# vanTeeffelenLab/ExTrack

Measured on AMD Instinct MI355X. Metric: log-likelihood evals/sec (1e6 tracks, 2-state, len=30), higher is better.
Workload: dtype f64

## Files before the change

### extrack_amd/csrc/xt_fast2.h

```cpp
#pragma once
#include "xt_kernel.h"

#define XT_F2_CHUNK 32
#ifndef XT_F2_RENORM
#define XT_F2_RENORM 3
#endif
#define XT_F2_WAVES 4

static inline bool xt_use_fast2(int S, int NS, int F, bool preds) { return S == 2 && NS == 1 && F >= 4 && F <= 7 && !preds; }

template <int F>
struct XtF2Geom {
    static constexpr int E = 1 << F;
    static constexpr int NG = E / 2;
    static constexpr int TPW = 64 / NG;
    static constexpr int EW = E * TPW;
};

template <int F>
XT_HD int xt_f2_swz(int w)
{
    const int c4[7] = {0x5, 0x12, 0x14, 0x2c, 0x4f, 0x41, 0x15};
    const int c6[7] = {0x15, 0x36, 0x67, 0x1c, 0x2, 0x1a, 0x16};
    const int c7[7] = {0x65, 0x72, 0x6, 0x69, 0x1c, 0x4, 0x5f};
    int s = 0;
    for (int j = 0; j < 7; ++j) {
        const int col = F == 6 ? c6[j] : (F == 7 ? c7[j] : c4[j]);
        s ^= ((w >> j) & 1) ? col : 0;
    }
    return s;
}

#define XT_F2_XCLAMP XT_TCLAMP
#define XT_F2_EXP_ENTRIES 1024
#define XT_F2_EXP_BYTES (XT_F2_EXP_ENTRIES * 8)
#define XT_F2_EXP_SCALE 1477.3197218702985
#define XT_F2_EXP_HI (-6.769015308236703e-04)
#define XT_F2_EXP_LO (-1.2691901263564344e-11)
#define XT_F2_EXP_C2 0.5000000047728719
XT_HD void xt_f2_exp_bits(double t, int& j, int& e)
{
    union {
        double d;
        unsigned long long u;
    } v;
    v.d = t;
    j = (int)(v.u & (XT_F2_EXP_ENTRIES - 1));
    e = (int)(unsigned int)(v.u >> 10);
}
XT_HD void xt_exp_tab_x2(double x0, double x1, double& p0, double& p1, int& j0, int& j1, int& e0, int& e1)
{
    x0 = x0 > XT_F2_XCLAMP ? x0 : XT_F2_XCLAMP;
    x1 = x1 > XT_F2_XCLAMP ? x1 : XT_F2_XCLAMP;
    const double t0 = xt_fma(x0, XT_F2_EXP_SCALE, XT_MAGIC);
    const double t1 = xt_fma(x1, XT_F2_EXP_SCALE, XT_MAGIC);
    const double k0 = t0 - XT_MAGIC;
    const double k1 = t1 - XT_MAGIC;
    double r0 = xt_fma(k0, XT_F2_EXP_HI, x0);
    double r1 = xt_fma(k1, XT_F2_EXP_HI, x1);
    r0 = xt_fma(k0, XT_F2_EXP_LO, r0);
    r1 = xt_fma(k1, XT_F2_EXP_LO, r1);
    double q0 = 1.66666666666666666667e-01, q1 = 1.66666666666666666667e-01;
#define XT_H2(C)              \
    q0 = xt_fma(q0, r0, (C)); \
    q1 = xt_fma(q1, r1, (C));
    XT_H2(XT_F2_EXP_C2)
    XT_H2(1.0)
    XT_H2(1.0)
#undef XT_H2
    p0 = q0;
    p1 = q1;
    xt_f2_exp_bits(t0, j0, e0);
    xt_f2_exp_bits(t1, j1, e1);
}
XT_HD void xt_exp_tab_x1(double x, double& p, int& j, int& e)
{
    x = x > XT_F2_XCLAMP ? x : XT_F2_XCLAMP;
    const double t = xt_fma(x, XT_F2_EXP_SCALE, XT_MAGIC);
    const double k = t - XT_MAGIC;
    double r = xt_fma(k, XT_F2_EXP_HI, x);
    r = xt_fma(k, XT_F2_EXP_LO, r);
#if defined(__HIP_DEVICE_COMPILE__)
    double q;
    asm("v_fma_f64 %0, %1, %2, %3" : "=v"(q) : "s"(1.66666666666666666667e-01), "v"(r), "v"(XT_F2_EXP_C2));
#else
    double q = xt_fma(1.66666666666666666667e-01, r, XT_F2_EXP_C2);
#endif
    q = xt_fma(q, r, 1.0);
    p = xt_fma(q, r, 1.0);
    xt_f2_exp_bits(t, j, e);
}
template <class Ctx>
XT_HD void xt_f2_build_exp_table(Ctx& cx, char* lds, int off, const double* T64)
{
    for (int i = cx.tid(); i < XT_F2_EXP_ENTRIES; i += cx.nthreads()) {
        const double sv = (double)(i & 15) * (XT_LN2 / 1024.0);
        double q = 1.0 / 5040.0;
        q = xt_fma(q, sv, 1.0 / 720.0);
        q = xt_fma(q, sv, 1.0 / 120.0);
        q = xt_fma(q, sv, 1.0 / 24.0);
        q = xt_fma(q, sv, 1.0 / 6.0);
        q = xt_fma(q, sv, 0.5);
        q = xt_fma(q, sv, 1.0);
        q = xt_fma(q, sv, 1.0);
        *(double*)(lds + off + i * 8) = T64[i >> 4] * q;
    }
}

template <int F, int D, int K>
struct XtF2State {
    int s01[F];
};

#define XT_F2_EXPB_OFF 1024
#define XT_F2_TAB_BYTES (1024 + XT_F2_EXP_BYTES)
#define XT_F2_T64_OFF ((XT_BLOB_HDR + XT_NTAB * 4) * 8)
#define XT_F2_NAN_OFF 832
#define XT_F2_ARR (XT_F2_WAVES * 128 * 8)
#define XT_F2_ZM0 XT_F2_TAB_BYTES
XT_HD int xt_f2_ze0(int D, int K) { return XT_F2_ZM0 + (1 + D + K) * XT_F2_ARR; }
XT_HD int xt_f2_pos0(int D, int K) { return xt_f2_ze0(D, K) + XT_F2_ARR; }
XT_HD int xt_f2_acc0(int D, int K, int KS, int tpw) { return xt_f2_pos0(D, K) + XT_F2_WAVES * tpw * XT_F2_CHUNK * (D + KS) * 8; }
XT_HD int xt_f2_block_bytes(int D, int K, int KS, int tpw) { return xt_f2_acc0(D, K, KS, tpw) + XT_F2_WAVES * 8 * 3 * 8; }

XT_HD int xt_opaque(int v)
{
#if defined(__HIP_DEVICE_COMPILE__)
    asm volatile("" : "+v"(v));
#endif
    return v;
}

template <class T>
XT_HD T& xt_at(char* lds, int byte_off)
{
#if defined(__HIP_DEVICE_COMPILE__)
    (void)lds;
    return *(__attribute__((address_space(3))) T*)(unsigned int)byte_off;
#else
    return *(T*)(lds + byte_off);
#endif
}
XT_HD void xt_f2_check_lds_base(char* lds)
{
#if defined(__HIP_DEVICE_COMPILE__)
    if ((unsigned int)(unsigned long long)(__attribute__((address_space(3))) char*)lds != 0u) __builtin_trap();
#else
    (void)lds;
#endif
}

template <int F, int D, int K, int H, bool ZF = false, bool LAZY = false>
XT_HD void xt_f2_step(char* lds, const XtF2State<F, D, K>& st, const double* c, const double* l2, const double* TT, const double* TD2)
{
    constexpr int ZEO = (1 + D + K) * XT_F2_ARR;
    const int pk = xt_opaque(st.s01[H]);
    const int a0 = pk & 0xffff, a1 = (int)((unsigned)pk >> 16);
    const double z0 = xt_at<double>(lds, a0), z1 = xt_at<double>(lds, a1);
    const int e0 = xt_at<int>(lds, a0 + ZEO), e1 = xt_at<int>(lds, a1 + ZEO);
    const int emax = e0 > e1 ? e0 : e1;
    const double w0 = xt_ldexp(z0, e0 - emax), w1 = xt_ldexp(z1, e1 - emax);
    const double W = w0 + w1;
    double M[D], U[K];
    for (int d = 0; d < D; ++d)
        M[d] = xt_fma(w1, xt_at<double>(lds, a1 + (1 + d) * XT_F2_ARR), w0 * xt_at<double>(lds, a0 + (1 + d) * XT_F2_ARR));
    for (int k = 0; k < K; ++k)
        U[k] = xt_fma(w1, xt_at<double>(lds, a1 + (1 + D + k) * XT_F2_ARR), w0 * xt_at<double>(lds, a0 + (1 + D + k) * XT_F2_ARR));
    const bool live = ZF ? true : W > 0.0;
    const double Ws = ZF ? W : (live ? W : 1.0);
    constexpr bool RN = !LAZY || (H % XT_F2_RENORM) == 0;
    const double Wm = RN ? xt_frexp_mant(W) : W;
    const int We = live ? (RN ? emax + xt_frexp_exp(W) : emax) : XT_EMIN;

    double Dq[2][K];
    for (int q = 0; q < 2; ++q)
        for (int k = 0; k < K; ++k) Dq[q][k] = xt_fma(Ws, l2[k] + TD2[q], U[k]);
    double rD[2][K], rW;
    if (K == 1) {
        const double d01 = Dq[0][0] * Dq[1][0];
        const double R = xt_rcp(Ws * d01);
        const double RW = R * Ws;
        rW = R * d01;
        rD[0][0] = RW * Dq[1][0];
        rD[1][0] = RW * Dq[0][0];
    } else {
        double f[2 * K + 1], pre[2 * K + 2], suf[2 * K + 2];
        f[0] = Ws;
        for (int q = 0; q < 2; ++q)
            for (int k = 0; k < K; ++k) f[1 + q * K + k] = Dq[q][k];
        pre[0] = 1.0;
        for (int i = 0; i < 2 * K + 1; ++i) pre[i + 1] = pre[i] * f[i];
        suf[2 * K + 1] = 1.0;
        for (int i = 2 * K; i >= 0; --i) suf[i] = suf[i + 1] * f[i];
        const double R = xt_rcp(pre[2 * K + 1]);
        rW = R * suf[1];
        for (int q = 0; q < 2; ++q)
            for (int k = 0; k < K; ++k) rD[q][k] = R * pre[1 + q * K + k] * suf[2 + q * K + k];
    }
    double dmW[D], dsqW = 0.0;
    for (int d = 0; d < D; ++d) {
        dmW[d] = xt_fma(c[d], Ws, -M[d]);
        if (K == 1) dsqW = xt_fma(dmW[d], dmW[d], dsqW);
    }
    double x[2], gf[2], tt[2][K];
    const double A = -0.5 * rW * dsqW;
    for (int q = 0; q < 2; ++q) {
        if (K == 1) {
            x[q] = A * rD[q][0];
            tt[q][0] = xt_fma(Ws, TD2[q], U[0]) * rD[q][0];
            gf[q] = xt_pow_half<D>(Ws * rD[q][0]);
        } else {
            double xx = 0.0, gg = 1.0;
            for (int d = 0; d < D; ++d) {
                xx = xt_fma(dmW[d] * dmW[d], rD[q][d], xx);
                tt[q][d] = xt_fma(Ws, TD2[q], U[d]) * rD[q][d];
                gg *= Ws * rD[q][d];
            }
            x[q] = xx * (-0.5 * rW);
            gf[q] = sqrt(gg);
        }
    }
    double p[2];
    int j[2], n[2];
    xt_exp_tab_x2(x[0], x[1], p[0], p[1], j[0], j[1], n[0], n[1]);
    for (int q = 0; q < 2; ++q) {
        const int aq = q ? a1 : a0;
        int en = We + n[q];
        const double tj = xt_at<double>(lds, XT_F2_EXPB_OFF + j[q] * 8);
        double zn = (Wm * TT[q]) * (gf[q] * tj) * p[q];
        if (!LAZY) {
            en += xt_frexp_exp(zn);
            zn = xt_frexp_mant(zn);
        }
        xt_at<double>(lds, aq) = zn;
        xt_at<int>(lds, aq + ZEO) = en > XT_EMIN ? en : XT_EMIN;
        for (int d = 0; d < D; ++d) xt_at<double>(lds, aq + (1 + d) * XT_F2_ARR) = xt_fma(dmW[d], tt[q][K == 1 ? 0 : d], M[d]) * rW;
        for (int k = 0; k < K; ++k) xt_at<double>(lds, aq + (1 + D + k) * XT_F2_ARR) = l2[k] * tt[q][k];
    }
}

template <int F, int D, int K, class Ctx>
// ... 232 lines not shown
```

### extrack_amd/csrc/xt_reg2.h

```cpp
#pragma once
#include "xt_fast2.h"
#include "xt_grad.h"


template <int F>
struct XtR2Geom {
    static constexpr int NGB = F - 1;
    static constexpr int NG = 1 << NGB;
    static constexpr int TPW = 64 / NG;
};
XT_HD constexpr int xt_r2_gbit(int F, int i) { return F == 7 ? i : (i < 2 ? i : i + 1); }
XT_HD constexpr int xt_r2_gmask(int F) { return F == 7 ? 63 : (F == 6 ? 0x3b : (F == 5 ? 0x1b : 0x0b)); }
template <int F>
XT_HD int xt_r2_slot(int lane)
{
    if (F == 7) return 0;
    int ts = (lane >> 2) & 1;
    if (F == 5) ts |= ((lane >> 5) & 1) << 1;
    if (F == 4) ts |= ((lane >> 4) & 3) << 1;
    return ts;
}

#define XT_R2_TAN0 XT_F2_TAB_BYTES
#define XT_R2_TB 36
// ... 124 lines not shown
        int en = We + n[q];
        const double tj = xt_at<double>(lds, XT_F2_EXPB_OFF + j[q] * 8);
        double zn = (Wm * TT[q]) * (gf[q] * tj) * p[q];
        if (!LAZY) {
            en += xt_frexp_exp(zn);
            zn = xt_frexp_mant(zn);
        }
        nz[q] = zn;
        ne[q] = en > XT_EMIN ? en : XT_EMIN;
        XT_UNROLL
        for (int d = 0; d < D; ++d) nm[q][d] = xt_fma(dmW[d], tt[q][K == 1 ? 0 : d], M[d]) * rW;
        XT_UNROLL
        for (int k = 0; k < K; ++k) nu[q][k] = l2[k] * tt[q][k];
    }

    double a0 = 0.0, a1 = 0.0, cm[D], cu[K], dn[D], Aq[2][K], rq[2][K];
    if (NP > 0) {
        a0 = w0 * rW;
        a1 = w1 * rW;
        const double aa = a0 * a1;
        XT_UNROLL
        for (int d = 0; d < D; ++d) {
            cm[d] = aa * (s.m[0][d] - s.m[1][d]);
            dn[d] = dmW[d] * rW;
        }
        XT_UNROLL
        for (int k = 0; k < K; ++k) cu[k] = aa * (s.u[0][k] - s.u[1][k]);
        XT_UNROLL
        for (int q = 0; q < 2; ++q)
            XT_UNROLL
            for (int k = 0; k < K; ++k) {
                rq[q][k] = Ws * rD[q][k];
                if (K == 1)
                    Aq[q][0] = -0.5 * rq[q][0] * xt_fma(-(dsqW * rW * rW), rq[q][0], (double)D);
                else
                    Aq[q][k] = -0.5 * rq[q][k] * xt_fma(-(dn[k] * dn[k]), rq[q][k], 1.0);
            }
    }
    cx.template pair_exchange<XB>(nz[0], nz[1]);
    cx.template pair_exchange_i32<XB>(ne[0], ne[1]);
    XT_UNROLL
    for (int d = 0; d < D; ++d) cx.template pair_exchange<XB>(nm[0][d], nm[1][d]);
    XT_UNROLL
    for (int k = 0; k < K; ++k) cx.template pair_exchange<XB>(nu[0][k], nu[1][k]);
    XT_UNROLL
    for (int q = 0; q < 2; ++q) {
        s.z[q] = nz[q];
        s.e[q] = ne[q];
        XT_UNROLL
        for (int d = 0; d < D; ++d) s.m[q][d] = nm[q][d];
        XT_UNROLL
        for (int k = 0; k < K; ++k) s.u[q][k] = nu[q][k];
    }
    if (NP > 0) {
        XT_UNROLL
        for (int pp = 0; pp < NP; ++pp) {
            if (!(VAR & 1)) xt_sched_fence();
            const int tb = XT_R2_TAN0 + pp * XT_R2_TB * 8;
            double dl[K];
            XT_UNROLL
            for (int k = 0; k < K; ++k) dl[k] = xt_at<double>(lds, tb + k * 8);
            const double del = s.rz[pp][0] - s.rz[pp][1];
            const double R = xt_fma(a0, s.rz[pp][0], a1 * s.rz[pp][1]);
            double dmb[D], dub[K];
            XT_UNROLL
            for (int d = 0; d < D; ++d) dmb[d] = xt_fma(cm[d], del, xt_fma(a0, s.dm[pp][0][d], a1 * s.dm[pp][1][d]));
            XT_UNROLL
            for (int k = 0; k < K; ++k) dub[k] = xt_fma(cu[k], del, xt_fma(a0, s.du[pp][0][k], a1 * s.du[pp][1][k]));
            double hd[K];
            if (K == 1) {
                hd[0] = 0.0;
                XT_UNROLL
                for (int d = 0; d < D; ++d) hd[0] = xt_fma(dn[d], dmb[d], hd[0]);
            } else {
                XT_UNROLL
                for (int d = 0; d < D; ++d) hd[d] = dn[d] * dmb[d];
            }
            double trz[2], tdm[2][D], tdu[2][K];
            XT_UNROLL
            for (int q = 0; q < 2; ++q) {
                const double dlT = xt_at<double>(lds, tb + tab + io[q]);
                const double dd2 = xt_at<double>(lds, tb + XT_R2_TAB0 + 4 * 32 + io[q]);
                double rzn = R + dlT, dtt[K];
                XT_UNROLL
                for (int k = 0; k < K; ++k) {
                    const double ds2 = dd2 + dub[k], dden = dl[k] + ds2;
                    dtt[k] = rq[q][k] * xt_fma(-tt[q][k], dden, ds2);
                    rzn = xt_fma(Aq[q][k], dden, rzn);
                    rzn = xt_fma(rq[q][k], hd[k], rzn);
                    tdu[q][k] = xt_fma(l2[k], dtt[k], dl[k] * tt[q][k]);
                }
                trz[q] = ZF ? rzn : (live ? rzn : 0.0);
                XT_UNROLL
                for (int d = 0; d < D; ++d) {
                    const int kk = K == 1 ? 0 : d;
                    tdm[q][d] = xt_fma(dn[d], dtt[kk], xt_fma(-tt[q][kk], dmb[d], dmb[d]));
                }
            }
            cx.template pair_exchange<XB>(trz[0], trz[1]);
            XT_UNROLL
            for (int d = 0; d < D; ++d) cx.template pair_exchange<XB>(tdm[0][d], tdm[1][d]);
            XT_UNROLL
            for (int k = 0; k < K; ++k) cx.template pair_exchange<XB>(tdu[0][k], tdu[1][k]);
            XT_UNROLL
            for (int q = 0; q < 2; ++q) {
                s.rz[pp][q] = trz[q];
                XT_UNROLL
                for (int d = 0; d < D; ++d) s.dm[pp][q][d] = tdm[q][d];
                XT_UNROLL
                for (int k = 0; k < K; ++k) s.du[pp][q][k] = tdu[q][k];
            }
        }
    }
}

#ifndef XT_R2_RC_H
#define XT_R2_RC_H 0
#endif
#define XT_R2_RC_NONE (-2147483647 - 1)
#define XT_R2_IO_BITS 5
template <int F, int H, class Ctx>
XT_HD int xt_r2_pack_io(int lane)
{
    constexpr int NGB = F - 1;
    if constexpr (H >= NGB) {
        return 0;
    } else {
        constexpr int XB = xt_r2_gbit(F, H), PB = xt_r2_gbit(F, (H + NGB - 1) % NGB);
        const int prev = (lane >> PB) & 1;
        const int qa = Ctx::template pair_natural<XB>() ? 0 : (lane >> XB) & 1;
        return ((prev * 2 + qa) * 8) << (XT_R2_IO_BITS * H) | xt_r2_pack_io<F, H + 1, Ctx>(lane);
    }
}
XT_HD void xt_r2_opaque_inplace(int& pk)
{
#if defined(__HIP_DEVICE_COMPILE__)
    asm volatile("" : "+v"(pk));
#else
    (void)pk;
#endif
}
template <class Ctx>
XT_HD int xt_r2_tid8(Ctx& cx)
{
#if defined(__HIP_DEVICE_COMPILE__)
    int o;
    asm volatile("v_lshlrev_b32 %0, 3, %1" : "=v"(o) : "v"(cx.tid()));
    return o;
#else
    return cx.tid() * 8;
#endif
}
template <int F, int D, int H, bool FIRST = false, class Ctx>
XT_HD void xt_r2_step_g(Ctx& cx, char* lds, XtR2Lane<D, 1, 0>& s, double (&lx)[2], int& pk, int tab, const double* c)
{
    constexpr int NGB = F - 1;
    constexpr int XB = xt_r2_gbit(F, H);
    xt_r2_opaque_inplace(pk);
    int io0 = (int)(((unsigned int)pk >> (XT_R2_IO_BITS * H)) & ((1u << XT_R2_IO_BITS) - 1u));
    xt_r2_opaque_inplace(io0);
    const int io[2] = {io0, io0 ^ 8};
    double TD2[2], LT[2];
    XT_UNROLL
    for (int q = 0; q < 2; ++q) {
        TD2[q] = xt_at<double>(lds, XT_R2_TAB0 + 4 * 32 + io[q]);
        LT[q] = xt_at<double>(lds, tab + XT_R2_LNT_REL + io[q]);
    }
    const double l2 = xt_at<double>(lds, 0), l22 = xt_at<double>(lds, XT_R2_GC_OFF + 8);

    double w0 = 1.0, w1 = 0.0, base = lx[0];
    if (!FIRST) {
        const double dl = lx[1] - lx[0];
        double p;
        int j, n;
        xt_exp_tab_x1(-fabs(dl), p, j, n);
        const double E = xt_ldexp(xt_at<double>(lds, XT_F2_EXPB_OFF + j * 8) * p, n);
        const bool up = dl > 0.0;
        w0 = s.z[0] * (up ? E : 1.0);
        w1 = s.z[1] * (up ? 1.0 : E);
        base = up ? lx[1] : lx[0];
    }
    const double Ws = FIRST ? 1.0 : w0 + w1;
    double M[D];
    XT_UNROLL
    for (int d = 0; d < D; ++d) M[d] = FIRST ? s.m[0][d] : xt_fma(w1, s.m[1][d], w0 * s.m[0][d]);
    const double V = FIRST ? s.u[0][0] : xt_fma(w1, s.u[1][0], w0 * s.u[0][0]);
    constexpr bool RN = !FIRST && (H % XT_F2_RENORM) == 0;
    const double Wm = FIRST ? s.z[0] : (RN ? xt_frexp_mant(Ws) : Ws);
    if (RN) base = xt_fma((double)xt_frexp_exp(Ws), XT_LN2, base);
    if (!FIRST && H == XT_R2_RC_H) {
        const int tid8 = xt_r2_tid8(cx);
        const int rc0 = xt_r2_rc0(D, 0, XtR2Geom<F>::TPW);
        const int cell = rc0 + (tid8 & ~(xt_r2_gmask(F) * 8));
        cx.atomic_max_i32(&xt_at<int>(lds, cell), (int)fmin(fmax(base, -1e9), 1e9));
        cx.wave_sync();
        const int sh = xt_at<int>(lds, cell);
        base -= (double)sh;
        xt_at<unsigned int>(lds, rc0 + XT_R2_RC_ARR + tid8) += (unsigned int)sh;
    }
    if (!FIRST && H == (XT_R2_RC_H + 1) % NGB) xt_at<int>(lds, xt_r2_rc0(D, 0, XtR2Geom<F>::TPW) + (xt_r2_tid8(cx) & ~(xt_r2_gmask(F) * 8))) = XT_R2_RC_NONE;

    const double Dq0 = xt_fma(Ws, TD2[0], V), Dq1 = xt_fma(Ws, TD2[1], V);
    const double R = xt_rcp3(Ws * (Dq0 * Dq1));
    const double h[2] = {R * Dq1, R * Dq0};
    const double l2W = FIRST ? l2 : l2 * Ws;
    double ed[D], esq = 0.0;
    XT_UNROLL
    for (int d = 0; d < D; ++d) {
        ed[d] = FIRST ? c[d] - M[d] : xt_fma(c[d], Ws, -M[d]);
        esq = xt_fma(ed[d], ed[d], esq);
    }
    const double Ah = -0.5 * esq;
    const double WmW = FIRST ? Wm : Wm * Ws;
    double ny[2], nl[2], nm[2][D], nv[2];
    XT_UNROLL
    for (int q = 0; q < 2; ++q) {
        const double k = l2W * h[q];
        ny[q] = D == 2 ? WmW * k : Wm * xt_pow_half<D>(FIRST ? k : Ws * k);
        nl[q] = xt_fma(Ah, h[q], LT[q]) + base;
        XT_UNROLL
        for (int d = 0; d < D; ++d) nm[q][d] = xt_fma(-ed[d], k, c[d]);
        nv[q] = xt_fma(-l2W, k, l22);
    }
    cx.template pair_exchange<XB>(ny[0], ny[1]);
    cx.template pair_exchange<XB>(nl[0], nl[1]);
    XT_UNROLL
    for (int d = 0; d < D; ++d) cx.template pair_exchange<XB>(nm[0][d], nm[1][d]);
    cx.template pair_exchange<XB>(nv[0], nv[1]);
    XT_UNROLL
    for (int q = 0; q < 2; ++q) {
        s.z[q] = ny[q];
        lx[q] = nl[q];
        XT_UNROLL
        for (int d = 0; d < D; ++d) s.m[q][d] = nm[q][d];
        s.u[q][0] = nv[q];
    }
}

template <int F, class Ctx>
XT_HD double xt_r2_gsum(Ctx& cx, double v)
{
    constexpr int NGB = F - 1;
    v += cx.template xor_f64<xt_r2_gbit(F, 0)>(v);
    v += cx.template xor_f64<xt_r2_gbit(F, 1)>(v);
    v += cx.template xor_f64<xt_r2_gbit(F, 2)>(v);
    if (NGB > 3) v += cx.template xor_f64<xt_r2_gbit(F, NGB > 3 ? 3 : 0)>(v);
    if (NGB > 4) v += cx.template xor_f64<xt_r2_gbit(F, NGB > 4 ? 4 : 0)>(v);
    if (NGB > 5) v += cx.template xor_f64<xt_r2_gbit(F, NGB > 5 ? 5 : 0)>(v);
    return v;
}
template <int F, class Ctx>
XT_HD int xt_r2_gmax(Ctx& cx, int v)
{
    constexpr int NGB = F - 1;
    auto mx = [](int a, int b) XT_INL { return a > b ? a : b; };
    v = mx(v, cx.template xor_i32<xt_r2_gbit(F, 0)>(v));
    v = mx(v, cx.template xor_i32<xt_r2_gbit(F, 1)>(v));
    v = mx(v, cx.template xor_i32<xt_r2_gbit(F, 2)>(v));
    if (NGB > 3) v = mx(v, cx.template xor_i32<xt_r2_gbit(F, NGB > 3 ? 3 : 0)>(v));
    if (NGB > 4) v = mx(v, cx.template xor_i32<xt_r2_gbit(F, NGB > 4 ? 4 : 0)>(v));
    if (NGB > 5) v = mx(v, cx.template xor_i32<xt_r2_gbit(F, NGB > 5 ? 5 : 0)>(v));
    return v;
}

template <int F, int D, int K, int NP, class Ctx, class GetPos>
XT_HD void xt_r2_chain(Ctx& cx, char* lds, XtR2Lane<D, K, NP>& s, int T, int stay_from, GetPos& getpos)
{
    constexpr int NGB = F - 1;
    const int lane = xt_opaque(cx.lane());
    double z = s.z[0];
    int e = s.e[0];
    XT_UNROLL
    for (int t = 1; t < NGB; ++t) {
        if (t > T) break;
        const int prev = (lane >> xt_r2_gbit(F, t == 1 ? NGB - 1 : t - 2)) & 1;
        const int q = (lane >> xt_r2_gbit(F, t - 1)) & 1;
        const int io = (prev * 2 + q) * 8;
        const double TT = xt_at<double>(lds, XT_R2_TAB0 + (t >= stay_from ? 32 : 0) + io);
        const double d2 = xt_at<double>(lds, XT_R2_TAB0 + 4 * 32 + io);
        double c[D], l2[K];
        getpos(t, c, l2);
        double tt[K], r[K], dm[D], x = 0.0, gf;
        XT_UNROLL
        for (int k = 0; k < K; ++k) {
            const double a = d2 + s.u[0][k];
            r[k] = NP == 0 ? xt_rcp3(l2[k] + a) : xt_rcp(l2[k] + a);
            tt[k] = a * r[k];
        }
        XT_UNROLL
        for (int d = 0; d < D; ++d) dm[d] = c[d] - s.m[0][d];
        if (K == 1) {
            XT_UNROLL
            for (int d = 0; d < D; ++d) x = xt_fma(dm[d], dm[d], x);
            x *= -0.5 * r[0];
            gf = xt_pow_half<D>(r[0]);
        } else {
            double gg = 1.0;
            XT_UNROLL
            for (int d = 0; d < D; ++d) {
                x = xt_fma(-0.5 * dm[d] * dm[d], r[d], x);
                gg *= r[d];
            }
            gf = sqrt(gg);
        }
        double p;
        int j, n;
        xt_exp_tab_x1(x, p, j, n);
        z = (z * TT) * (gf * xt_at<double>(lds, XT_F2_EXPB_OFF + j * 8)) * p;
        e += n;
        XT_UNROLL
        for (int d = 0; d < D; ++d) s.m[0][d] = xt_fma(dm[d], tt[K == 1 ? 0 : d], s.m[0][d]);
        XT_UNROLL
        for (int k = 0; k < K; ++k) s.u[0][k] = l2[k] * tt[k];
    }
    int dummy = 0;
    XT_UNROLL
    for (int i = 0; i < NGB - 1; ++i)
        if (i >= T) dummy |= 1 << xt_r2_gbit(F, i);
    const bool live = (lane & dummy) == 0;
    s.z[0] = live ? xt_frexp_mant(z) : 0.0;
    s.e[0] = live ? e + xt_frexp_exp(z) : XT_EMIN;
}

template <int F, int D, int K, int NP, int VAR = 0, class Ctx>
XT_HD void xt_r2_body(const XtKernelArgs& a, const XtGradArgs& ga, Ctx& cx)
{
    int lb, nb;
    const XtBucketDesc b = xt_bind_bucket(a, cx.block(), cx.nblocks(), lb, nb);
    typedef XtR2Geom<F> Gm;
    constexpr int NGB = Gm::NGB, TPW = Gm::TPW;
    constexpr int GMASK = xt_r2_gmask(F);
    const int lane = cx.lane();
    const int wib = NP == 0 ? cx.uniform(cx.wave_in_block()) : cx.wave_in_block();
    const int nwb = cx.waves_per_block();
    const int L = b.L;
    const int KS = a.locerr_mode ? a.KS : 0;
    double* smem = cx.smem();
    char* lds = (char*)smem;

    const int ntab = xt_tab_doubles(2, 2);
    for (int i = cx.tid(); i < ntab; i += cx.nthreads()) smem[i] = xt_blob_ptr(a)[i];
    if (NP > 0)
        for (int i = cx.tid(); i < NP * XT_R2_TB; i += cx.nthreads()) xt_at<double>(lds, XT_R2_TAN0 + i * 8) = ga.dblob[i];
    const int NU = NP > 0 ? ga.NU : 0, NPT = NP + NU;
    for (int i = cx.tid(); i < NU * XT_R2_TB; i += cx.nthreads()) xt_at<double>(lds, XT_R2_TAN0 + (NP * XT_R2_TB + i) * 8) = ga.udblob[i];
    cx.sync();
    xt_f2_check_lds_base(lds);
    xt_f2_build_exp_table(cx, lds, XT_F2_EXPB_OFF, (const double*)(lds + XT_F2_T64_OFF));
    const bool gform = NP == 0 && K == 1 && a.well_scaled == 2 && a.locerr_mode == 0;
    if constexpr (NP == 0 && K == 1) {
        if (gform && cx.tid() < 10) {
            const int i = cx.tid();
            const double l2 = smem[0];
            if (i < 8)
                xt_at<double>(lds, XT_R2_LNT_OFF + i * 8) = log(smem[XT_BLOB_HDR + i]) - 0.5 * D * log(l2);
            else
                xt_at<double>(lds, XT_R2_GC_OFF + (i - 8) * 8) = i == 8 ? -0.5 / l2 : 2.0 * l2;
        }
    }
    cx.sync();
    const double* hdr = smem;

    const int ts = xt_r2_slot<F>(lane);
    const bool leader = (lane & GMASK) == 0;
    const int tlast = L - 1;
    const int stay_from = a.min_len > 2 ? a.min_len : 2;
    const int vfin = (b.isBL ? 2 : 0) + (tlast >= stay_from ? 1 : 0);
    double l2g[K];
    XT_UNROLL
    for (int k = 0; k < K; ++k) l2g[k] = hdr[k];
    int pk = xt_r2_pack_io<F, 0, Ctx>(lane);
    const bool well_scaled = a.well_scaled != 0;
    const bool chain = NP == 0 && well_scaled;

    double* pos = (double*)(lds + xt_r2_pos0(NPT)) + wib * TPW * XT_F2_CHUNK * (D + KS);
    double* sig = pos + TPW * XT_F2_CHUNK * D;
    const int posb = NP == 0 ? xt_opaque(xt_r2_pos0(0) + (wib * TPW * XT_F2_CHUNK * (D + KS) + ts * XT_F2_CHUNK * D) * 8) : 0;
    double* accp = (double*)(lds + xt_r2_acc0(NPT, D, KS, TPW)) + (wib * 8 + ts) * (NPT + 3);
    auto accb = [&]() XT_INL { return xt_r2_acc0(0, D, KS, TPW) + (wib * 8 + xt_r2_slot<F>(xt_opaque(cx.lane()))) * 24; };
    auto rcacc = [&]() XT_INL { return xt_r2_rc0(D, KS, TPW) + XT_R2_RC_ARR + xt_opaque(cx.tid()) * 8; };
    auto rcsum = [&]() XT_INL { return xt_r2_rc0(D, KS, TPW) + 2 * XT_R2_RC_ARR + (wib * 8 + xt_r2_slot<F>(xt_opaque(cx.lane()))) * 8; };
    if (leader) {
        if (NP == 0) {
            const int ab = accb();
            xt_at<double>(lds, ab) = 1.0;
            xt_at<double>(lds, ab + 8) = 0.0;
            xt_at<double>(lds, ab + 16) = 0.0;
            xt_at<double>(lds, rcsum()) = 0.0;
        } else {
            for (int i = 0; i < NPT + 1; ++i) accp[i] = 0.0;
        }
    }

    const int64_t nbatch = (b.N + TPW - 1) / TPW;
    const int64_t W0 = (int64_t)lb * nwb + wib, NW = (int64_t)nb * nwb;
    for (int64_t batch = W0; batch < nbatch; batch += NW) {
        const int64_t trk = batch * TPW + ts;
        const bool act = trk < b.N;

        auto stage = [&](int p0) XT_INL {
            cx.wave_sync();
            for (int i = lane; i < TPW * XT_F2_CHUNK * D; i += 64) {
                const int t_ = i / (XT_F2_CHUNK * D), r = i - t_ * (XT_F2_CHUNK * D);
                const int64_t tk = batch * TPW + t_;
                const int64_t tkc = tk < b.N ? tk : b.N - 1;
                const int pp = p0 + r / D;
                if (pp < L) {
                    const double v = b.tracks[(tkc * L + p0) * D + r];
                    pos[i] = v;
                    if (v != v) xt_at<int>(lds, XT_F2_NAN_OFF + (wib * 8 + t_) * 4) = 1;
                }
            }
            if (KS)
                for (int i = lane; i < TPW * XT_F2_CHUNK * KS; i += 64) {
                    const int t_ = i / (XT_F2_CHUNK * KS), r = i - t_ * (XT_F2_CHUNK * KS);
                    const int64_t tk = batch * TPW + t_;
                    const int64_t tkc = tk < b.N ? tk : b.N - 1;
                    const int pp = p0 + r / KS;
                    if (pp < L) {
                        const double v = b.sigma[(tkc * L + p0) * KS + r];
                        sig[i] = v;
                        if (v != v) xt_at<int>(lds, XT_F2_NAN_OFF + (wib * 8 + t_) * 4) = 1;
                    }
                }
            cx.wave_sync();
        };
        auto getpos = [&](int t, double* c, double* l2) XT_INL {
            const int r = t & (XT_F2_CHUNK - 1);
            XT_UNROLL
            for (int d = 0; d < D; ++d) c[d] = NP == 0 ? xt_at<double>(lds, posb + (r * D + d) * 8) : pos[(ts * XT_F2_CHUNK + r) * D + d];
            if (KS == 0) {
                XT_UNROLL
                for (int k = 0; k < K; ++k) l2[k] = xt_at<double>(lds, k * 8);
            } else {
                XT_UNROLL
                for (int k = 0; k < K; ++k) {
                    double sg = sig[(ts * XT_F2_CHUNK + r) * KS + (KS == 1 ? 0 : k)];
                    if (a.locerr_mode == 2) {
                        sg = xt_fma(sg, hdr[3], hdr[4]);
                        sg = sg < 1e-6 ? 1e-6 : sg;
                    }
                    l2[k] = sg * sg;
                }
            }
        };

        XtR2Lane<D, K, NP> s;
        double lx[2] = {0.0, 0.0};
#define XT_R2_PHASE(H, ZF_, LAZY_)                                                                     \
    if (NGB > (H) && t <= tend2 && ph == (H)) {                                                        \
        double c[D], l2[K];                                                                            \
        getpos(t, c, l2);                                                                              \
        xt_r2_step<F, D, K, NP, ((H) < NGB ? (H) : 0), ZF_, LAZY_, VAR>(cx, lds, s, XT_R2_TABSEL, c, l2);   \
        ++t;                                                                                           \
        ph = (H) + 1 == NGB ? 0 : (H) + 1;                                                             \
    }
#define XT_R2_PHASE_G(H)                                                                               \
    if (NGB > (H) && t <= tend2 && ph == (H)) {                                                        \
        double c[D], l2[K];                                                                            \
        getpos(t, c, l2);                                                                              \
        xt_r2_step_g<F, D, ((H) < NGB ? (H) : 0)>(cx, lds, s, lx, pk, XT_R2_TABSEL, c);                    \
        ++t;                                                                                           \
        ph = (H) + 1 == NGB ? 0 : (H) + 1;                                                             \
    }
#define XT_R2_PHASES(ZF_, LAZY_) \
    XT_R2_PHASE(0, ZF_, LAZY_)   \
    XT_R2_PHASE(1, ZF_, LAZY_)   \
    XT_R2_PHASE(2, ZF_, LAZY_)   \
    XT_R2_PHASE(3, ZF_, LAZY_)   \
    XT_R2_PHASE(4, ZF_, LAZY_)   \
    XT_R2_PHASE(5, ZF_, LAZY_)
#define XT_R2_TABSEL tab
        auto run_steps = [&](int& t, int tend, int tab) XT_INL {
            int ph = (t - 1) % NGB;
            const int tend2 = tend;
            if (!well_scaled) {
                while (t <= tend2) { XT_R2_PHASES(false, false) }
                return;
            }
            if constexpr (NP == 0 && K == 1) {
                if (gform) {
                    while (t <= tend2) {
                        XT_R2_PHASE_G(0)
                        XT_R2_PHASE_G(1)
                        XT_R2_PHASE_G(2)
                        XT_R2_PHASE_G(3)
                        XT_R2_PHASE_G(4)
                        XT_R2_PHASE_G(5)
                    }
                    return;
                }
            }
            while (t <= tend2) { XT_R2_PHASES(true, true) }
        };
#undef XT_R2_TABSEL
#define XT_R2_TABSEL (XT_R2_TAB0 + (t >= stay_from ? 32 : 0))
        auto run_steps_g = [&](int& t, int tend) XT_INL {
            int ph = (t - 1) % NGB;
            const int tend2 = tend;
            if (well_scaled) {
                while (t <= tend2) { XT_R2_PHASES(false, true) }
            } else {
                while (t <= tend2) { XT_R2_PHASES(false, false) }
            }
        };
#undef XT_R2_TABSEL
#undef XT_R2_PHASES
#undef XT_R2_PHASE_G
#undef XT_R2_PHASE

        XtAcc tot;
        tot.clear();
        double gacc[NP ? NP : 1];
        double uacc[XT_R2_MAXU];
        int fe = XT_EMIN;
        int t = 1;
        if (lane < 8) xt_at<int>(lds, XT_F2_NAN_OFF + (wib * 8 + lane) * 4) = 0;
        if (NP == 0) {
            xt_at<int>(lds, rcacc()) = 0;
            xt_at<int>(lds, rcacc() - XT_R2_RC_ARR) = XT_R2_RC_NONE;
        }
        for (int p0 = 0; p0 < L; p0 += XT_F2_CHUNK) {
            stage(p0);
            if (p0 == 0) {
                constexpr int NBIT = xt_r2_gbit(F, NGB - 1);
                double c0[D], l20[K];
                getpos(0, c0, l20);
                const bool live0 = chain || (lane & (GMASK & ~(1 << NBIT))) == 0;
                const int s0 = (lane >> NBIT) & 1;
                s.z[0] = live0 ? hdr[8 + s0] : 0.0;
                s.e[0] = live0 ? 0 : XT_EMIN;
                s.z[1] = 0.0;
                s.e[1] = XT_EMIN;
                XT_UNROLL
                for (int q = 0; q < 2; ++q) {
                    XT_UNROLL
                    for (int d = 0; d < D; ++d) s.m[q][d] = c0[d];
                    XT_UNROLL
                    for (int k = 0; k < K; ++k) s.u[q][k] = l20[k];
                }
                XT_UNROLL
                for (int pp = 0; pp < NP; ++pp) {
                    const int tb = XT_R2_TAN0 + pp * XT_R2_TB * 8;
                    s.rz[pp][0] = live0 ? xt_at<double>(lds, tb + (8 + s0) * 8) : 0.0;
                    s.rz[pp][1] = 0.0;
                    XT_UNROLL
                    for (int q = 0; q < 2; ++q) {
                        XT_UNROLL
                        for (int d = 0; d < D; ++d) s.dm[pp][q][d] = 0.0;
                        XT_UNROLL
                        for (int k = 0; k < K; ++k) s.du[pp][q][k] = xt_at<double>(lds, tb + k * 8);
                    }
                }
                if constexpr (NP == 0) {
                    if (chain) {
                        const int T = L - 2 < NGB - 1 ? L - 2 : NGB - 1;
                        xt_r2_chain<F>(cx, lds, s, T, stay_from, getpos);
                        if (L - 2 >= F - 1) {
                            double c[D], l2[K];
                            getpos(F - 1, c, l2);
                            bool first_done = false;
                            if constexpr (K == 1) {
                                if (gform) {
                                    s.u[0][0] += l2[0];
                                    lx[0] = (double)s.e[0] * XT_LN2;
                                    xt_r2_step_g<F, D, NGB - 1, true>(cx, lds, s, lx, pk, XT_R2_TAB0 + (F - 1 >= stay_from ? 32 : 0), c);
                                    s.e[0] = s.e[1] = 0;
                                    first_done = true;
                                }
                            }
                            if (!first_done) xt_r2_step<F, D, K, NP, NGB - 1, true, true, VAR, true>(cx, lds, s, XT_R2_TAB0 + (F - 1 >= stay_from ? 32 : 0), c, l2);
                            t = F;
                        } else {
                            t = L - 1 > 1 ? L - 1 : 1;
                        }
                    }
                }
            }
            const int tend = (L - 2 < p0 + XT_F2_CHUNK - 1) ? L - 2 : p0 + XT_F2_CHUNK - 1;
            if (NP == 0) {
                run_steps(t, tend < stay_from - 1 ? tend : stay_from - 1, XT_R2_TAB0);
                run_steps(t, tend, XT_R2_TAB0 + 32);
            } else {
                run_steps_g(t, tend);
            }
            if (tlast < p0 || tlast >= p0 + XT_F2_CHUNK) continue;
            double cl[D], l2l[K];
            getpos(tlast, cl, l2l);
            if constexpr (NP == 0 && K == 1) {
                if (gform && L - 2 >= F - 1) l2l[0] = 0.0;
            }
            const int hp = (tlast - 2 + NGB) % NGB;
            const int pbit = (F == 7 || hp < 2) ? hp : hp + 1;
            const int prev = (lane >> pbit) & 1;
            double wm[4], rr[4][K], dq[2][D], dsqQ[2];
            int we[4];
            if constexpr (NP == 0 && K == 1) {
                double dn[4];
                XT_UNROLL
                for (int i = 0; i < 4; ++i) dn[i] = xt_at<double>(lds, XT_R2_TAB0 + 4 * 32 + (prev * 2 + (i & 1)) * 8) + s.u[i >> 1][0] + l2l[0];
                const double p01 = dn[0] * dn[1], p23 = dn[2] * dn[3];
                const double R = xt_rcp3(p01 * p23);
                const double r01 = R * p23, r23 = R * p01;
                rr[0][0] = r01 * dn[1];
                rr[1][0] = r01 * dn[0];
                rr[2][0] = r23 * dn[3];
                rr[3][0] = r23 * dn[2];
            }
            XT_UNROLL
            for (int Q = 0; Q < 2; ++Q) {
                dsqQ[Q] = 0.0;
                XT_UNROLL
                for (int d = 0; d < D; ++d) {
                    dq[Q][d] = cl[d] - s.m[Q][d];
                    dsqQ[Q] = xt_fma(dq[Q][d], dq[Q][d], dsqQ[Q]);
                }
                double x[2], gf[2];
                XT_UNROLL
                for (int q = 0; q < 2; ++q) {
                    const double d2 = xt_at<double>(lds, XT_R2_TAB0 + 4 * 32 + (prev * 2 + q) * 8);
                    if (K == 1) {
                        double r;
                        if constexpr (NP == 0) {
                            r = rr[Q * 2 + q][0];
                        } else {
                            r = xt_rcp(d2 + s.u[Q][0] + l2l[0]);
                            rr[Q * 2 + q][0] = r;
                        }
                        x[q] = -0.5 * dsqQ[Q] * r;
                        if constexpr (NP == 0) x[q] += lx[Q];
                        gf[q] = xt_pow_half<D>(r);
                    } else {
                        double xx = 0.0, gg = 1.0;
                        XT_UNROLL
                        for (int d = 0; d < D; ++d) {
                            const double r = NP == 0 ? xt_rcp3(d2 + s.u[Q][d] + l2l[d]) : xt_rcp(d2 + s.u[Q][d] + l2l[d]);
                            rr[Q * 2 + q][d] = r;
                            xx = xt_fma(-0.5 * dq[Q][d] * dq[Q][d], r, xx);
                            gg *= r;
                        }
                        x[q] = xx;
                        gf[q] = sqrt(gg);
                    }
                }
                double p[2];
                int j[2], n[2];
                xt_exp_tab_x2(x[0], x[1], p[0], p[1], j[0], j[1], n[0], n[1]);
                XT_UNROLL
                for (int q = 0; q < 2; ++q) {
                    const double tf = xt_at<double>(lds, XT_R2_TAB0 + vfin * 32 + (prev * 2 + q) * 8);
                    wm[Q * 2 + q] = s.z[Q] * tf * gf[q] * xt_at<double>(lds, XT_F2_EXPB_OFF + j[q] * 8) * p[q];
                    we[Q * 2 + q] = s.e[Q] + n[q];
                    tot.add(wm[Q * 2 + q], we[Q * 2 + q]);
                }
            }
            fe = xt_r2_gmax<F>(cx, tot.m != 0.0 ? tot.e : XT_EMIN);
            if (NP > 0) {
                double ws[4];
                XT_UNROLL
                for (int i = 0; i < 4; ++i) ws[i] = wm[i] != 0.0 ? xt_ldexp(wm[i], we[i] - fe) : 0.0;
                XT_UNROLL
                for (int pp = 0; pp < NP; ++pp) {
                    const int tb = XT_R2_TAN0 + pp * XT_R2_TB * 8;
                    double dl[K];
                    XT_UNROLL
                    for (int k = 0; k < K; ++k) dl[k] = xt_at<double>(lds, tb + k * 8);
                    double acc = 0.0;
                    XT_UNROLL
                    for (int Q = 0; Q < 2; ++Q) {
                        XT_UNROLL
                        for (int q = 0; q < 2; ++q) {
                            const double dlT = xt_at<double>(lds, tb + XT_R2_TAB0 + vfin * 32 + (prev * 2 + q) * 8);
                            const double dd2 = xt_at<double>(lds, tb + XT_R2_TAB0 + 4 * 32 + (prev * 2 + q) * 8);
                            double rel = s.rz[pp][Q] + dlT;
                            if (K == 1) {
                                const double r = rr[Q * 2 + q][0];
                                const double dden = dd2 + s.du[pp][Q][0] + dl[0];
                                double ddsq = 0.0;
                                XT_UNROLL
                                for (int d = 0; d < D; ++d) ddsq = xt_fma(-2.0 * dq[Q][d], s.dm[pp][Q][d], ddsq);
                                rel -= 0.5 * r * (D * dden + ddsq - dsqQ[Q] * r * dden);
                            } else {
                                XT_UNROLL
                                for (int d = 0; d < D; ++d) {
                                    const double r = rr[Q * 2 + q][d];
                                    const double dden = dd2 + s.du[pp][Q][d] + dl[d];
                                    rel -= 0.5 * r * (dden - 2.0 * dq[Q][d] * s.dm[pp][Q][d] - dq[Q][d] * dq[Q][d] * r * dden);
                                }
                            }
                            acc = xt_fma(ws[Q * 2 + q], ws[Q * 2 + q] != 0.0 ? rel : 0.0, acc);
                        }
                    }
                    gacc[pp] = acc;
                }
                XT_UNROLL
                for (int u = 0; u < XT_R2_MAXU; ++u) {
                    double acc = 0.0;
                    if (u < NU) {
                        const int tb = XT_R2_TAN0 + (NP + u) * XT_R2_TB * 8;
                        XT_UNROLL
                        for (int i = 0; i < 4; ++i) acc = xt_fma(ws[i], xt_at<double>(lds, tb + XT_R2_TAB0 + vfin * 32 + (prev * 2 + (i & 1)) * 8), acc);
                    }
                    uacc[u] = acc;
                }
            }
        }
        double sum = xt_r2_gsum<F>(cx, tot.m != 0.0 ? xt_ldexp(tot.m, tot.e - fe) : 0.0);
        const bool poisoned = xt_at<int>(lds, XT_F2_NAN_OFF + (wib * 8 + ts) * 4) != 0;
        if (poisoned) sum = NAN;
        if (NP == 0) {
            const int lz = xt_opaque(cx.lane());
            const int64_t trk = batch * TPW + xt_r2_slot<F>(lz);
            if (trk < b.N && (lz & GMASK) == 0) {
                const double rcs = (double)xt_at<int>(lds, rcacc());
                if (b.ll_out) b.ll_out[trk] = log(sum) + (double)fe * XT_LN2 + b.ll_const + rcs;
                xt_at<double>(lds, rcsum()) += rcs;
                const int ab = accb();
                const double pm = xt_at<double>(lds, ab) * xt_frexp_mant(sum);
                double acce = xt_at<double>(lds, ab + 8) + (double)(fe + xt_frexp_exp(sum) + xt_frexp_exp(pm));
                if (sum == 0.0) acce = -INFINITY;
                xt_at<double>(lds, ab) = xt_frexp_mant(pm);
                xt_at<double>(lds, ab + 8) = acce;
                xt_at<double>(lds, ab + 16) += 1.0;
            }
        } else {
            const double rs = 1.0 / sum;
            double gsum[NP ? NP : 1];
            XT_UNROLL
            for (int pp = 0; pp < NP; ++pp) gsum[pp] = xt_r2_gsum<F>(cx, gacc[pp]);
            double usum[XT_R2_MAXU];
            XT_UNROLL
            for (int u = 0; u < XT_R2_MAXU; ++u) usum[u] = u < NU ? xt_r2_gsum<F>(cx, uacc[u]) : 0.0;
            if (act && leader) {
                const double ll = log(sum) + (double)fe * XT_LN2 + b.ll_const;
                if (b.ll_out) b.ll_out[trk] = ll;
                accp[0] += ll;
                XT_UNROLL
                for (int pp = 0; pp < NP; ++pp) accp[1 + pp] += gsum[pp] * rs;
                double* const srow = b.scores_out ? b.scores_out + trk * ga.score_ld : nullptr;
                if (srow) {
                    XT_UNROLL
                    for (int pp = 0; pp < NP; ++pp) srow[ga.score_col0 + pp] = gsum[pp] * rs;
                }
                const int nsteps = L - 2 > 0 ? L - 2 : 0;
                const int n1 = nsteps >= stay_from ? nsteps - stay_from + 1 : 0, n0 = nsteps - n1;
                XT_UNROLL
                for (int u = 0; u < XT_R2_MAXU; ++u)
                    if (u < NU) {
                        const int tb = XT_R2_TAN0 + (NP + u) * XT_R2_TB * 8;
                        const double rzu = xt_at<double>(lds, tb + 8 * 8) + n0 * xt_at<double>(lds, tb + XT_R2_TAB0) + n1 * xt_at<double>(lds, tb + XT_R2_TAB0 + 32);
                        accp[1 + NP + u] += usum[u] * rs + rzu;
                        if (srow) srow[ga.score_ucol0 + u] = usum[u] * rs + rzu;
                    }
            }
        }
        cx.wave_sync();
    }

    cx.sync();
    if (NP == 0) {
        if (leader) {
            const double* ac = &xt_at<double>(lds, accb());
            smem[wib * TPW + ts] = ac[2] > 0.0 ? log(ac[0]) + ac[1] * XT_LN2 + ac[2] * b.ll_const + xt_at<double>(lds, rcsum()) : 0.0;
        }
        cx.sync();
        if (cx.tid() == 0) {
            double sacc = 0.0;
            for (int i = 0; i < nwb * TPW; ++i) sacc += smem[i];
            a.partials[cx.block()] = sacc;
        }
    } else {
        const double* acc0 = (const double*)(lds + xt_r2_acc0(NPT, D, KS, TPW));
        for (int col = cx.tid(); col < NPT + 1; col += cx.nthreads()) {
            double sacc = 0.0;
            for (int w = 0; w < nwb; ++w)
                for (int i = 0; i < TPW; ++i) sacc += acc0[(w * 8 + i) * (NPT + 3) + col];
            ga.gpartials[(int64_t)cx.block() * (NPT + 1) + col] = sacc;
        }
    }
}
```

Before: 465.4.

## Reparameterize gform recursion in scaled log space with position differences

Rewrites the 2-state forward step to carry lambda = -2·log-weight and residuals relative to the next position (pre-differenced track coordinates) instead of absolute means. This removes per-step FMAs and multiplies (the c*Ws-M residual, the -0.5 scaling) and adds a dedicated gform chain warm-up, xt_r2_chain_g, that runs in the same representation. The exp helper is changed to take a doubled argument, and the rescale counters and log tables are stored in the new scale. The main risk is numeric: the sign and scale changes in the rescaling atomics and the final log-likelihood correction must stay exactly consistent.

```diff
diff --git a/extrack_amd/csrc/xt_fast2.h b/extrack_amd/csrc/xt_fast2.h
--- a/extrack_amd/csrc/xt_fast2.h
+++ b/extrack_amd/csrc/xt_fast2.h
@@ -87,6 +87,23 @@
     double q = xt_fma(1.66666666666666666667e-01, r, XT_F2_EXP_C2);
 #endif
     q = xt_fma(q, r, 1.0);
+    p = xt_fma(q, r, 1.0);
+    xt_f2_exp_bits(t, j, e);
+}
+XT_HD void xt_exp_tab_half_x1(double x2, double& p, int& j, int& e)
+{
+    x2 = x2 > 2.0 * XT_F2_XCLAMP ? x2 : 2.0 * XT_F2_XCLAMP;
+    const double t = xt_fma(x2, 0.5 * XT_F2_EXP_SCALE, XT_MAGIC);
+    const double k = t - XT_MAGIC;
+    double r = xt_fma(k, 2.0 * XT_F2_EXP_HI, x2);
+    r = xt_fma(k, 2.0 * XT_F2_EXP_LO, r);
+#if defined(__HIP_DEVICE_COMPILE__)
+    double q;
+    asm("v_fma_f64 %0, %1, %2, %3" : "=v"(q) : "s"(1.66666666666666666667e-01 / 8.0), "v"(r), "v"(0.25 * XT_F2_EXP_C2));
+#else
+    double q = xt_fma(1.66666666666666666667e-01 / 8.0, r, 0.25 * XT_F2_EXP_C2);
+#endif
+    q = xt_fma(q, r, 0.5);
     p = xt_fma(q, r, 1.0);
     xt_f2_exp_bits(t, j, e);
 }
diff --git a/extrack_amd/csrc/xt_reg2.h b/extrack_amd/csrc/xt_reg2.h
--- a/extrack_amd/csrc/xt_reg2.h
+++ b/extrack_amd/csrc/xt_reg2.h
@@ -300,7 +300,7 @@
 #endif
 }
 template <int F, int D, int H, bool FIRST = false, class Ctx>
-XT_HD void xt_r2_step_g(Ctx& cx, char* lds, XtR2Lane<D, 1, 0>& s, double (&lx)[2], int& pk, int tab, const double* c)
+XT_HD void xt_r2_step_g(Ctx& cx, char* lds, XtR2Lane<D, 1, 0>& s, double (&lam)[2], int& pk, int tab, const double* dc)
 {
     constexpr int NGB = F - 1;
     constexpr int XB = xt_r2_gbit(F, H);
@@ -316,35 +316,38 @@
     }
     const double l2 = xt_at<double>(lds, 0), l22 = xt_at<double>(lds, XT_R2_GC_OFF + 8);
 
-    double w0 = 1.0, w1 = 0.0, base = lx[0];
+    double w0 = 1.0, w1 = 0.0, base = lam[0];
     if (!FIRST) {
-        const double dl = lx[1] - lx[0];
+        const double dl = lam[1] - lam[0];
         double p;
         int j, n;
-        xt_exp_tab_x1(-fabs(dl), p, j, n);
+        xt_exp_tab_half_x1(-fabs(dl), p, j, n);
         const double E = xt_ldexp(xt_at<double>(lds, XT_F2_EXPB_OFF + j * 8) * p, n);
-        const bool up = dl > 0.0;
+        const bool up = dl < 0.0;
         w0 = s.z[0] * (up ? E : 1.0);
         w1 = s.z[1] * (up ? 1.0 : E);
-        base = up ? lx[1] : lx[0];
+        base = up ? lam[1] : lam[0];
     }
     const double Ws = FIRST ? 1.0 : w0 + w1;
-    double M[D];
-    XT_UNROLL
-    for (int d = 0; d < D; ++d) M[d] = FIRST ? s.m[0][d] : xt_fma(w1, s.m[1][d], w0 * s.m[0][d]);
+    double ed[D], esq = 0.0;
+    XT_UNROLL
+    for (int d = 0; d < D; ++d) {
+        ed[d] = FIRST ? s.m[0][d] : xt_fma(w1, s.m[1][d], w0 * s.m[0][d]);
+        esq = xt_fma(ed[d], ed[d], esq);
+    }
     const double V = FIRST ? s.u[0][0] : xt_fma(w1, s.u[1][0], w0 * s.u[0][0]);
     constexpr bool RN = !FIRST && (H % XT_F2_RENORM) == 0;
     const double Wm = FIRST ? s.z[0] : (RN ? xt_frexp_mant(Ws) : Ws);
-    if (RN) base = xt_fma((double)xt_frexp_exp(Ws), XT_LN2, base);
+    if (RN) base = xt_fma((double)xt_frexp_exp(Ws), -2.0 * XT_LN2, base);
     if (!FIRST && H == XT_R2_RC_H) {
         const int tid8 = xt_r2_tid8(cx);
         const int rc0 = xt_r2_rc0(D, 0, XtR2Geom<F>::TPW);
         const int cell = rc0 + (tid8 & ~(xt_r2_gmask(F) * 8));
-        cx.atomic_max_i32(&xt_at<int>(lds, cell), (int)fmin(fmax(base, -1e9), 1e9));
+        cx.atomic_max_i32(&xt_at<int>(lds, cell), (int)fmin(fmax(-base, -1e9), 1e9));
         cx.wave_sync();
-        const int sh = xt_at<int>(lds, cell);
-        base -= (double)sh;
-        xt_at<unsigned int>(lds, rc0 + XT_R2_RC_ARR + tid8) += (unsigned int)sh;
+        const int nsh = xt_at<int>(lds, cell);
+        base += (double)nsh;
+        xt_at<unsigned int>(lds, rc0 + XT_R2_RC_ARR + tid8) -= (unsigned int)nsh;
     }
     if (!FIRST && H == (XT_R2_RC_H + 1) % NGB) xt_at<int>(lds, xt_r2_rc0(D, 0, XtR2Geom<F>::TPW) + (xt_r2_tid8(cx) & ~(xt_r2_gmask(F) * 8))) = XT_R2_RC_NONE;
 
@@ -352,37 +355,68 @@
     const double R = xt_rcp3(Ws * (Dq0 * Dq1));
     const double h[2] = {R * Dq1, R * Dq0};
     const double l2W = FIRST ? l2 : l2 * Ws;
-    double ed[D], esq = 0.0;
-    XT_UNROLL
-    for (int d = 0; d < D; ++d) {
-        ed[d] = FIRST ? c[d] - M[d] : xt_fma(c[d], Ws, -M[d]);
-        esq = xt_fma(ed[d], ed[d], esq);
-    }
-    const double Ah = -0.5 * esq;
     const double WmW = FIRST ? Wm : Wm * Ws;
-    double ny[2], nl[2], nm[2][D], nv[2];
+    double ny[2], nl[2], nr[2][D], nv[2];
     XT_UNROLL
     for (int q = 0; q < 2; ++q) {
         const double k = l2W * h[q];
         ny[q] = D == 2 ? WmW * k : Wm * xt_pow_half<D>(FIRST ? k : Ws * k);
-        nl[q] = xt_fma(Ah, h[q], LT[q]) + base;
-        XT_UNROLL
-        for (int d = 0; d < D; ++d) nm[q][d] = xt_fma(-ed[d], k, c[d]);
+        nl[q] = xt_fma(esq, h[q], LT[q]) + base;
+        XT_UNROLL
+        for (int d = 0; d < D; ++d) nr[q][d] = xt_fma(ed[d], k, dc[d]);
         nv[q] = xt_fma(-l2W, k, l22);
     }
     cx.template pair_exchange<XB>(ny[0], ny[1]);
     cx.template pair_exchange<XB>(nl[0], nl[1]);
     XT_UNROLL
-    for (int d = 0; d < D; ++d) cx.template pair_exchange<XB>(nm[0][d], nm[1][d]);
+    for (int d = 0; d < D; ++d) cx.template pair_exchange<XB>(nr[0][d], nr[1][d]);
     cx.template pair_exchange<XB>(nv[0], nv[1]);
     XT_UNROLL
     for (int q = 0; q < 2; ++q) {
         s.z[q] = ny[q];
-        lx[q] = nl[q];
-        XT_UNROLL
-        for (int d = 0; d < D; ++d) s.m[q][d] = nm[q][d];
+        lam[q] = nl[q];
+        XT_UNROLL
+        for (int d = 0; d < D; ++d) s.m[q][d] = nr[q][d];
         s.u[q][0] = nv[q];
     }
+}
+
+template <int F, int D, class Ctx, class GetPos>
+XT_HD void xt_r2_chain_g(Ctx& cx, char* lds, XtR2Lane<D, 1, 0>& s, double (&lam)[2], int T, int stay_from, GetPos& getpos)
+{
+    constexpr int NGB = F - 1;
+    const int lane = xt_opaque(cx.lane());
+    const double l2 = xt_at<double>(lds, 0), l22 = xt_at<double>(lds, XT_R2_GC_OFF + 8);
+    double y = s.z[0], la = lam[0], v = s.u[0][0];
+    XT_UNROLL
+    for (int t = 1; t < NGB; ++t) {
+        if (t > T) break;
+        const int prev = (lane >> xt_r2_gbit(F, t == 1 ? NGB - 1 : t - 2)) & 1;
+        const int q = (lane >> xt_r2_gbit(F, t - 1)) & 1;
+        const int io = (prev * 2 + q) * 8;
+        const double LT = xt_at<double>(lds, XT_R2_LNT_OFF + (t >= stay_from ? 32 : 0) + io);
+        const double d2 = xt_at<double>(lds, XT_R2_TAB0 + 4 * 32 + io);
+        double dc[D], l2u[1];
+        getpos(t, dc, l2u);
+        const double rd = xt_rcp3(d2 + v);
+        const double g = l2 * rd;
+        double rsq = 0.0;
+        XT_UNROLL
+        for (int d = 0; d < D; ++d) rsq = xt_fma(s.m[0][d], s.m[0][d], rsq);
+        y *= xt_pow_half<D>(g);
+        la = xt_fma(rsq, rd, la + LT);
+        v = xt_fma(-l2, g, l22);
+        XT_UNROLL
+        for (int d = 0; d < D; ++d) s.m[0][d] = xt_fma(s.m[0][d], g, dc[d]);
+    }
+    int dummy = 0;
+    XT_UNROLL
+    for (int i = 0; i < NGB - 1; ++i)
+        if (i >= T) dummy |= 1 << xt_r2_gbit(F, i);
+    const bool live = (lane & dummy) == 0;
+    s.z[0] = live ? xt_frexp_mant(y) : 0.0;
+    lam[0] = xt_fma((double)xt_frexp_exp(y), -2.0 * XT_LN2, la);
+    s.u[0][0] = v;
 }
 
 template <int F, class Ctx>
@@ -501,7 +535,7 @@
             const int i = cx.tid();
             const double l2 = smem[0];
             if (i < 8)
-                xt_at<double>(lds, XT_R2_LNT_OFF + i * 8) = log(smem[XT_BLOB_HDR + i]) - 0.5 * D * log(l2);
+                xt_at<double>(lds, XT_R2_LNT_OFF + i * 8) = -2.0 * (log(smem[XT_BLOB_HDR + i]) - 0.5 * D * log(l2));
             else
                 xt_at<double>(lds, XT_R2_GC_OFF + (i - 8) * 8) = i == 8 ? -0.5 / l2 : 2.0 * l2;
         }
@@ -554,8 +588,14 @@
                 const int64_t tkc = tk < b.N ? tk : b.N - 1;
                 const int pp = p0 + r / D;
                 if (pp < L) {
-                    const double v = b.tracks[(tkc * L + p0) * D + r];
-                    pos[i] = v;
+                    const double* const src = b.tracks + (tkc * L + p0) * D + r;
+                    const double v = src[0];
+                    if constexpr (NP == 0 && K == 1) {
+                        const double vn = src[pp + 1 < L ? D : 0];
+                        pos[i] = gform ? vn - v : v;
+                    } else {
+                        pos[i] = v;
+                    }
                     if (v != v) xt_at<int>(lds, XT_F2_NAN_OFF + (wib * 8 + t_) * 4) = 1;
                 }
             }
@@ -594,7 +634,7 @@
         };
 
         XtR2Lane<D, K, NP> s;
-        double lx[2] = {0.0, 0.0};
+        double lam[2] = {0.0, 0.0};
 #define XT_R2_PHASE(H, ZF_, LAZY_)                                                                     \
     if (NGB > (H) && t <= tend2 && ph == (H)) {                                                        \
         double c[D], l2[K];                                                                            \
@@ -607,7 +647,7 @@
     if (NGB > (H) && t <= tend2 && ph == (H)) {                                                        \
         double c[D], l2[K];                                                                            \
         getpos(t, c, l2);                                                                              \
-        xt_r2_step_g<F, D, ((H) < NGB ? (H) : 0)>(cx, lds, s, lx, pk, XT_R2_TABSEL, c);                    \
+        xt_r2_step_g<F, D, ((H) < NGB ? (H) : 0)>(cx, lds, s, lam, pk, XT_R2_TABSEL, c);                   \
         ++t;                                                                                           \
         ph = (H) + 1 == NGB ? 0 : (H) + 1;                                                             \
     }
@@ -687,6 +727,9 @@
                     XT_UNROLL
                     for (int k = 0; k < K; ++k) s.u[q][k] = l20[k];
                 }
+                if constexpr (NP == 0 && K == 1) {
+                    if (gform) s.u[0][0] = s.u[1][0] = 2.0 * l20[0];
+                }
                 XT_UNROLL
                 for (int pp = 0; pp < NP; ++pp) {
                     const int tb = XT_R2_TAN0 + pp * XT_R2_TB * 8;
@@ -703,17 +746,22 @@
                 if constexpr (NP == 0) {
                     if (chain) {
                         const int T = L - 2 < NGB - 1 ? L - 2 : NGB - 1;
-                        xt_r2_chain<F>(cx, lds, s, T, stay_from, getpos);
+                        bool chain_done = false;
+                        if constexpr (K == 1) {
+                            if (gform) {
+                                xt_r2_chain_g<F>(cx, lds, s, lam, T, stay_from, getpos);
+                                s.e[0] = s.e[1] = 0;
+                                chain_done = true;
+                            }
+                        }
+                        if (!chain_done) xt_r2_chain<F>(cx, lds, s, T, stay_from, getpos);
                         if (L - 2 >= F - 1) {
                             double c[D], l2[K];
                             getpos(F - 1, c, l2);
                             bool first_done = false;
                             if constexpr (K == 1) {
                                 if (gform) {
-                                    s.u[0][0] += l2[0];
-                                    lx[0] = (double)s.e[0] * XT_LN2;
-                                    xt_r2_step_g<F, D, NGB - 1, true>(cx, lds, s, lx, pk, XT_R2_TAB0 + (F - 1 >= stay_from ? 32 : 0), c);
-                                    s.e[0] = s.e[1] = 0;
+                                    xt_r2_step_g<F, D, NGB - 1, true>(cx, lds, s, lam, pk, XT_R2_TAB0 + (F - 1 >= stay_from ? 32 : 0), c);
                                     first_done = true;
                                 }
                             }
@@ -736,7 +784,7 @@
             double cl[D], l2l[K];
             getpos(tlast, cl, l2l);
             if constexpr (NP == 0 && K == 1) {
-                if (gform && L - 2 >= F - 1) l2l[0] = 0.0;
+                if (gform) l2l[0] = 0.0;
             }
             const int hp = (tlast - 2 + NGB) % NGB;
             const int pbit = (F == 7 || hp < 2) ? hp : hp + 1;
@@ -761,6 +809,9 @@
                 XT_UNROLL
                 for (int d = 0; d < D; ++d) {
                     dq[Q][d] = cl[d] - s.m[Q][d];
+                    if constexpr (NP == 0 && K == 1) {
+                        if (gform) dq[Q][d] = s.m[Q][d];
+                    }
                     dsqQ[Q] = xt_fma(dq[Q][d], dq[Q][d], dsqQ[Q]);
                 }
                 double x[2], gf[2];
@@ -775,8 +826,10 @@
                             r = xt_rcp(d2 + s.u[Q][0] + l2l[0]);
                             rr[Q * 2 + q][0] = r;
                         }
-                        x[q] = -0.5 * dsqQ[Q] * r;
-                        if constexpr (NP == 0) x[q] += lx[Q];
+                        if constexpr (NP == 0)
+                            x[q] = -0.5 * xt_fma(dsqQ[Q], r, lam[Q]);
+                        else
+                            x[q] = -0.5 * dsqQ[Q] * r;
                         gf[q] = xt_pow_half<D>(r);
                     } else {
                         double xx = 0.0, gg = 1.0;
@@ -860,7 +913,7 @@
             const int lz = xt_opaque(cx.lane());
             const int64_t trk = batch * TPW + xt_r2_slot<F>(lz);
             if (trk < b.N && (lz & GMASK) == 0) {
-                const double rcs = (double)xt_at<int>(lds, rcacc());
+                const double rcs = -0.5 * (double)xt_at<int>(lds, rcacc());
                 if (b.ll_out) b.ll_out[trk] = log(sum) + (double)fe * XT_LN2 + b.ll_const + rcs;
                 xt_at<double>(lds, rcsum()) += rcs;
                 const int ab = accb();
```

After: 471.7, median of 6. +1.4%, better.
